# CoderWZW/ARLib

Hardware: AMD Instinct MI355X
Metric: BPR-train interactions/sec (LightGCN d=64 L=3 + BPR + Adam, B=2048) (higher is better)
Workload: dtype f32

## Files before the change

### arlib_amd/csrc/arl_kernels.hip

```cpp
#include <hip/hip_runtime.h>
#include <stdint.h>
#include <math.h>
#include <stdio.h>
#include "arlib_amd.h"
#include "arl_stream.h"
#include "arl_ordered.h"
#include <type_traits>
#include <algorithm>
#include <vector>

namespace {

constexpr int kWave = 64;
constexpr int kBlock = 256;
constexpr int kWavesPerBlock = kBlock / kWave;

__device__ __forceinline__ float wave_sum(float v) {
#pragma unroll
    for (int off = 32; off > 0; off >>= 1) v += __shfl_xor(v, off);
    return v;
}

__device__ __forceinline__ void fma4(float4 &a, float s, const float4 &x) {
    a.x = fmaf(s, x.x, a.x); a.y = fmaf(s, x.y, a.y); a.z = fmaf(s, x.z, a.z); a.w = fmaf(s, x.w, a.w);
// ... 368 lines not shown
    S->cap = (int)cap;
    S->piece_row = w + cap * d;
    S->meta = S->piece_row + cap;
    S->offs = S->meta + 2;
    return true;
}

__global__ __launch_bounds__(kBlock) void tables_sum_kernel(LayerPtrs L, long long n4, float alpha, float4 *__restrict__ out) {
    for (long long t = (long long)blockIdx.x * kBlock + threadIdx.x; t < n4; t += (long long)gridDim.x * kBlock) {
        float4 a = reinterpret_cast<const float4 *>(L.p[0])[t];
        for (int k = 1; k < L.n; ++k) a = add4(a, reinterpret_cast<const float4 *>(L.p[k])[t]);
        out[t] = make_float4(alpha * a.x, alpha * a.y, alpha * a.z, alpha * a.w);
    }
}

__global__ __launch_bounds__(kBlock) void mark_rows_kernel(uint8_t *__restrict__ flags, const int32_t *__restrict__ idx, int n, int value) {
    const int t = blockIdx.x * kBlock + threadIdx.x;
    if (t < n) flags[idx[t]] = (uint8_t)value;
}
__global__ __launch_bounds__(kBlock) void mark_bits_kernel(uint32_t *__restrict__ bits, const int32_t *__restrict__ idx, int n, int set) {
    const int t = blockIdx.x * kBlock + threadIdx.x;
    if (t >= n) return;
    const int i = idx[t];
    if (set) atomicOr(bits + (i >> 5), 1u << (i & 31));
    else atomicAnd(bits + (i >> 5), ~(1u << (i & 31)));
}
__global__ __launch_bounds__(kBlock) void zero_rows_kernel(float *__restrict__ dst, const int32_t *__restrict__ idx, int n, int d) {
    const int lane = threadIdx.x & 63;
    const int t = blockIdx.x * kWavesPerBlock + (threadIdx.x >> 6);
    if (t >= n) return;
    float *o = dst + (size_t)idx[t] * d;
    for (int k = lane; k < d; k += kWave) o[k] = 0.f;
}

template <class RowOf>
__device__ __forceinline__ void stage_rows(int32_t *srows, int c0, int c1, RowOf rowof) {
    for (int j = threadIdx.x; j < c1 - c0; j += kBlock) srows[j] = (int32_t)rowof(c0 + j);
    __syncthreads();
}

__global__ __launch_bounds__(kBlock) void rows_mark_dups_kernel(uint32_t *__restrict__ bits, uint32_t *__restrict__ dup, const int32_t *__restrict__ idx, int n,
                                                                 const float *__restrict__ row_scale) {
    const int t = blockIdx.x * kBlock + threadIdx.x;
    if (t >= n) return;
    if (row_scale && row_scale[t] == 0.f) return;
    const int row = idx[t];
    const uint32_t m = 1u << (row & 31);
    if (atomicOr(bits + (row >> 5), m) & m) atomicOr(dup + (row >> 5), m);
}

template <bool MARK>
__global__ __launch_bounds__(kBlock) void rows_add_ordered_kernel(float *__restrict__ dst, uint8_t *__restrict__ flags, uint32_t *__restrict__ bits,
                                                                   const int32_t *__restrict__ idx, int c0, int c1, int d,
                                                                   const float *__restrict__ src, float scale, const float *__restrict__ row_scale,
                                                                   const uint32_t *__restrict__ dup) {
    extern __shared__ int32_t srows[];
    const int lane = threadIdx.x & 63;
    const int t = c0 + blockIdx.x * kWavesPerBlock + (threadIdx.x >> 6);
    const bool valid = t < c1 && !(row_scale && row_scale[t] == 0.f);
    const int row = valid ? idx[t] : 0;
    float *o = dst + (size_t)row * d;
    const bool fast = valid && dup && !((dup[row >> 5] >> (row & 31)) & 1u);
    if (fast) {
        const float sc = row_scale ? scale * row_scale[t] : scale;
        const float *s = src + (size_t)t * d;
        for (int k = lane; k < d; k += kWave) {
#pragma clang fp contract(off)
            const float c = sc * s[k];
            o[k] = o[k] + c;
        }
        if (MARK && lane == 0) flags[row] = 1;
    }
    if (!__syncthreads_or(valid && !fast)) return;
    stage_rows(srows, c0, c1, [&](int j) { return (row_scale && row_scale[j] == 0.f) ? -1 : idx[j]; });
    if (!valid || fast) return;
    for (int k0 = 0; k0 < d; k0 += 256) {
        float acc[4];
#pragma unroll
        for (int i = 0; i < 4; ++i) { const int k = k0 + 64 * i + lane; acc[i] = k < d ? o[k] : 0.f; }
        const bool owner = ordered_scan_lds_groups(srows, c0, c1, t, row, lane, [&](unsigned long long m, int g0) {
#pragma clang fp contract(off)
            while (m) {
                int tt[4]; float x[4][4], sc[4];
#pragma unroll
                for (int q = 0; q < 4; ++q) {
                    tt[q] = -1;
                    if (m) { tt[q] = g0 + __ffsll((long long)m) - 1; m &= m - 1ull; }
                }
#pragma unroll
                for (int q = 0; q < 4; ++q) {
                    if (tt[q] < 0) continue;
                    const float *s = src + (size_t)tt[q] * d;
                    sc[q] = row_scale ? scale * row_scale[tt[q]] : scale;
#pragma unroll
                    for (int i = 0; i < 4; ++i) { const int k = k0 + 64 * i + lane; x[q][i] = k < d ? s[k] : 0.f; }
                }
#pragma unroll
                for (int q = 0; q < 4; ++q) {
                    if (tt[q] < 0) continue;
#pragma unroll
                    for (int i = 0; i < 4; ++i) { const float c = sc[q] * x[q][i]; acc[i] = acc[i] + c; }
                }
            }
        });
        if (!owner) return;
#pragma unroll
        for (int i = 0; i < 4; ++i) { const int k = k0 + 64 * i + lane; if (k < d) o[k] = acc[i]; }
    }
    if (MARK && lane == 0) {
        flags[row] = 1;
        atomicOr(bits + (row >> 5), 1u << (row & 31));
    }
}
__global__ __launch_bounds__(kBlock) void batch_rows_clear_kernel(float *__restrict__ G, uint8_t *__restrict__ flags, uint32_t *__restrict__ bits,
                                                                   const int32_t *__restrict__ idx, int n, int d, uint32_t *__restrict__ dup) {
    const int lane = threadIdx.x & 63;
    const int t = blockIdx.x * kWavesPerBlock + (threadIdx.x >> 6);
    if (t >= n) return;
    const int row = idx[t];
    float *o = G + (size_t)row * d;
    for (int k = lane; k < d; k += kWave) o[k] = 0.f;
    if (lane == 0) {
        flags[row] = 0;
        atomicAnd(bits + (row >> 5), ~(1u << (row & 31)));
        if (dup) atomicAnd(dup + (row >> 5), ~(1u << (row & 31)));
    }
}

template <int MODE>
int launch_spmm(const arl_csr *A, const float *X, int64_t d, const Epi &ep, hipStream_t st, const uint32_t *xflags = nullptr) {
    if (!A || !X || (A->n_rows > 0 && !A->rowptr) || (A->nnz > 0 && (!A->col || !A->val))) return ARL_E_NULL;
    if (d <= 0 || d > 256 || (d & 3)) return ARL_E_DIM;
    if (A->n_rows < 0 || A->n_rows > 0x7fffffffll || A->nnz > 0x7fffffffll || A->n_chunks > 0x7fffffffll) return ARL_E_RANGE;
    if (A->n_chunks > 0 && (!A->chunk_row || !A->chunk_begin || !A->chunk_end || !A->partial || A->chunk <= 0)) return ARL_E_NULL;
    if (A->n_long > 0 && (!A->long_row || !A->long_first || !A->long_count)) return ARL_E_NULL;
    if ((A->n_chunks > 0) != (A->n_long > 0)) return ARL_E_ARG;
    if (A->n_rows == 0 && A->n_chunks == 0) return ARL_OK;
    CsrDev D;
    D.n_rows = (int)A->n_rows; D.rowptr = A->rowptr; D.col = A->col; D.val = A->val;
    D.chunk = A->chunk; D.n_chunks = (int)A->n_chunks; D.chunk_row = A->chunk_row; D.chunk_begin = A->chunk_begin;
    D.chunk_end = A->chunk_end; D.n_long = (int)A->n_long; D.long_row = A->long_row; D.long_first = A->long_first;
    D.long_count = A->long_count; D.partial = A->partial;
    D.row_tasks = xflags ? reinterpret_cast<const int4 *>(A->row_tasks) : nullptr;
    const long long tasks = (long long)D.n_rows + D.n_chunks;
    const unsigned grid = (unsigned)((tasks + kWavesPerBlock - 1) / kWavesPerBlock);
    const unsigned grid_long = (unsigned)((D.n_long + kWavesPerBlock - 1) / kWavesPerBlock);
    const int di = (int)d;
#define ARL_SPMM_CASE(LPRV)                                                                              \
    do {                                                                                                 \
        if (xflags) hipLaunchKernelGGL((spmm_rows_masked_gpr_kernel<LPRV, MODE>), dim3((unsigned)((tasks + kWavesPerBlock * (kWave / LPRV) - 1) / (kWavesPerBlock * (kWave / LPRV)))), dim3(kBlock), 0, st, D, X, di, ep, xflags); \
        else hipLaunchKernelGGL((spmm_rows_kernel<LPRV, MODE>), dim3(grid), dim3(kBlock), 0, st, D, X, di, ep); \
        ARL_LAUNCH_CHECK();                                                                              \
        if (D.n_long > 0) {                                                                              \
            hipLaunchKernelGGL((spmm_long_rows_kernel<LPRV, MODE>), dim3(grid_long), dim3(kBlock), 0, st, D, di, ep); \
            ARL_LAUNCH_CHECK();                                                                          \
        }                                                                                                \
    } while (0)
    if (d <= 16) ARL_SPMM_CASE(4);
    else if (d <= 32) ARL_SPMM_CASE(8);
    else if (d <= 64) ARL_SPMM_CASE(16);
    else if (d <= 128) ARL_SPMM_CASE(32);
    else ARL_SPMM_CASE(64);
#undef ARL_SPMM_CASE
    return ARL_OK;
}

typedef float f32x32v __attribute__((ext_vector_type(32)));

struct BlockedDev {
    int n_waves;
    const int32_t *wave_ptr;
    const int32_t *wave_rows;
    const int32_t *rec_col;
    const float *rec_val;
    float *partial;
    const uint32_t *xbits;
};

template <int MODE> constexpr int kEpiLoads = MODE == EPI_ADAM ? 4 : 1;
template <int MODE> constexpr int kEpiStores = MODE == EPI_ADAM ? 3 : MODE == EPI_LAYERSUM ? 2 : 1;

template <int MODE>
__device__ __forceinline__ float *spmm_epilogue_table(const Epi &ep, int s) {
    if (MODE == EPI_AXPBY) return ep.Y;
    if (MODE == EPI_LAYERSUM) return s == 0 ? ep.Y : ep.S;
    return s == 0 ? ep.P : s == 1 ? ep.M : ep.V;
}

template <int MODE, int CPL>
__device__ __forceinline__ void spmm_epilogue_math(const Epi &ep, bool zr, float rs, const float *a, const float (&in)[kEpiLoads<MODE>][CPL],
                                                   float (&out)[kEpiStores<MODE>][CPL]) {
#pragma unroll
    for (int c = 0; c < CPL; ++c) {
#pragma clang fp contract(off)
        if constexpr (MODE == EPI_AXPBY) {
            float y = (ep.rscale ? ep.alpha * rs : ep.alpha) * a[c];
            if (zr) y = fmaf(ep.beta, in[0][c], y);
            out[0][c] = y;
        } else if constexpr (MODE == EPI_LAYERSUM) {
            out[0][c] = a[c];
            out[1][c] = in[0][c] + a[c];
        } else {
            float g = ep.alpha * a[c];
            if (zr) g = fmaf(ep.beta, in[0][c], g);
            float p = in[1][c], m = in[2][c], v = in[3][c];
            m = m + (g - m) * ep.w1;
            v = fmaf(ep.w2 * g, g, v * ep.b2);
            const float denom = sqrtf(v) / ep.bc2_sqrt + ep.eps;
            p = fmaf(-ep.step_size, m / denom, p);
            out[0][c] = p; out[1][c] = m; out[2][c] = v;
        }
    }
}

template <int MODE, int CPL, int LD>
__device__ __forceinline__ void spmm_epilogue1(const Epi &ep, int row, bool zr, float rs, int lane, const float *a) {
    const size_t o = (size_t)row * LD;
    const unsigned lo = lane * CPL;
    float in[kEpiLoads<MODE>][CPL], out[kEpiStores<MODE>][CPL];
#pragma unroll
    for (int c = 0; c < CPL; ++c) {
        in[0][c] = 0.f;
        if constexpr (MODE == EPI_LAYERSUM) in[0][c] = (ep.S_in + o)[lo + c];
        else if (zr) in[0][c] = (ep.Z + o)[lo + c];
        if constexpr (MODE == EPI_ADAM) { in[1][c] = (ep.P + o)[lo + c]; in[2][c] = (ep.M + o)[lo + c]; in[3][c] = (ep.V + o)[lo + c]; }
    }
    spmm_epilogue_math<MODE, CPL>(ep, zr, rs, a, in, out);
#pragma unroll
    for (int s = 0; s < kEpiStores<MODE>; ++s) {
        if (MODE == EPI_LAYERSUM && s == 0 && !ep.Y) continue;
        float *dst = spmm_epilogue_table<MODE>(ep, s) + o;
#pragma unroll
        for (int c = 0; c < CPL; ++c) {
            if (MODE == EPI_AXPBY) __builtin_nontemporal_store(out[s][c], dst + (lo + c));
            else dst[lo + c] = out[s][c];
        }
    }
}

template <int MODE, int K, int CPL, int LD>
__device__ __forceinline__ void spmm_group_load(const Epi &ep, int my_row, unsigned zmask, int safe_row, int r0, int lane, float (&in)[K][kEpiLoads<MODE>][CPL]) {
    const unsigned lo = lane * CPL;
    const size_t so = (size_t)safe_row * LD;
    if constexpr (MODE != EPI_LAYERSUM) {
#pragma unroll
        for (int i = 0; i < K; ++i)
#pragma unroll
            for (int c = 0; c < CPL; ++c) in[i][0][c] = 0.f;
        if (ep.Z) {
#pragma unroll
            for (int i = 0; i < K; ++i) {
                const int row = __builtin_amdgcn_readlane(my_row, r0 + i);
                const float *z = ((zmask >> (r0 + i)) & 1u) ? ep.Z + (size_t)row * LD : ep.Z + so;
#pragma unroll
                for (int c = 0; c < CPL; ++c) in[i][0][c] = z[lo + c];
            }
        }
    }
    if constexpr (MODE != EPI_AXPBY) {
#pragma unroll
        for (int i = 0; i < K; ++i) {
            const int row = __builtin_amdgcn_readlane(my_row, r0 + i);
            const size_t o = (size_t)row * LD;
#pragma unroll
            for (int c = 0; c < CPL; ++c) {
                if constexpr (MODE == EPI_LAYERSUM) in[i][0][c] = (row >= 0 ? ep.S_in + o : ep.S_in + so)[lo + c];
                else {
                    in[i][1][c] = (row >= 0 ? ep.P + o : ep.P + so)[lo + c];
                    in[i][2][c] = (row >= 0 ? ep.M + o : ep.M + so)[lo + c];
                    in[i][3][c] = (row >= 0 ? ep.V + o : ep.V + so)[lo + c];
                }
            }
        }
    }
}

template <int MODE, int K, int CPL, int LD>
__device__ __forceinline__ void spmm_group_store(const Epi &ep, float *partial, int my_row, int r0, int lane, const float (&a)[K][CPL],
                                                 const float (&out)[K][kEpiStores<MODE>][CPL]) {
    const unsigned lo = lane * CPL;
#pragma unroll
    for (int s = 0; s < kEpiStores<MODE>; ++s) {
        if (MODE == EPI_LAYERSUM && s == 0 && !ep.Y) continue;
        float *tab = spmm_epilogue_table<MODE>(ep, s);
#pragma unroll
        for (int i = 0; i < K; ++i) {
            const int row = __builtin_amdgcn_readlane(my_row, r0 + i);
            const bool plain = row >= 0;
            float *dst = plain ? tab + (size_t)row * LD : partial + (size_t)(plain ? 0 : -row - 2) * (64 * CPL);
#pragma unroll
            for (int c = 0; c < CPL; ++c) {
                const float y = plain ? out[i][s][c] : a[i][c];
                if (MODE == EPI_AXPBY) __builtin_nontemporal_store(y, dst + (lo + c));
                else dst[lo + c] = y;
            }
        }
    }
}

template <int UNR, bool MASKED> constexpr bool kEpiGrouped = MASKED || UNR == 16;
template <int MODE, bool MASKED> constexpr int kEpiGroup = MODE == EPI_ADAM ? 2 : MASKED ? 8 : 4;

constexpr int kMaskedUnr = 8;

constexpr int kMaxMergedSets = 4;
struct BlockedSetsDev {
    int n;
    int block_end[kMaxMergedSets];
    BlockedDev s[kMaxMergedSets];
};

template <int RPW, int MODE, int UNR, int CPL, int LD = 64 * CPL, bool MASKED = false, typename PLAN = BlockedDev>
__global__ __launch_bounds__(kBlock) void spmm_blocked64_kernel(PLAN plan, const float *__restrict__ X, Epi ep) {
    static_assert(RPW == 16 || RPW == 32, "accumulators are 32-register vectors");
    static_assert(CPL == 1 || CPL == 2, "d = 64 (one column per lane) or d = 128 (two adjacent columns per lane)");
    const int lane = threadIdx.x & 63;
    BlockedDev P;
    int w;
    if constexpr (std::is_same<PLAN, BlockedSetsDev>::value) {
        P = plan.s[0];
        int b0 = 0;
#pragma unroll
        for (int i = 1; i < kMaxMergedSets; ++i)
            if (i < plan.n && (int)blockIdx.x >= plan.block_end[i - 1]) { P = plan.s[i]; b0 = plan.block_end[i - 1]; }
        w = ((int)blockIdx.x - b0) * (blockDim.x >> 6) + (threadIdx.x >> 6);
    } else {
        P = plan;
        w = blockIdx.x * (blockDim.x >> 6) + (threadIdx.x >> 6);
    }
    if (w >= P.n_waves) return;
    f32x32v acc[CPL];
#pragma unroll
    for (int c = 0; c < CPL; ++c)
#pragma unroll
        for (int r = 0; r < 32; ++r) acc[c][r] = 0.f;
    const int begin = P.wave_ptr[w], end = P.wave_ptr[w + 1];
    constexpr bool GROUPED = kEpiGrouped<UNR, MASKED>;
    int my_row = -1;
    if (GROUPED && lane < RPW) my_row = P.wave_rows[(size_t)w * RPW + lane];
    const float *xl = X + lane * CPL;
    if (MASKED) {
        int c0 = 0, c1 = 0; unsigned w0 = 0;
        if (begin < end) c0 = __builtin_nontemporal_load(P.rec_col + begin + lane);
        if (begin + 64 < end) c1 = __builtin_nontemporal_load(P.rec_col + begin + 64 + lane);
        if (begin < end) w0 = P.xbits[((unsigned)c0 & 0xffffffu) >> 5];
        for (int base = begin; base < end; base += 64) {
            const int c_cur = c0; const unsigned w_cur = w0;
            c0 = c1;
            if (base + 128 < end) c1 = __builtin_nontemporal_load(P.rec_col + base + 128 + lane);
            if (base + 64 < end) w0 = P.xbits[((unsigned)c0 & 0xffffffu) >> 5];
            unsigned long long hits = __ballot((w_cur >> (c_cur & 31)) & 1u);
            while (hits) {
                float x[kMaskedUnr][CPL], vs[kMaskedUnr]; int cs[kMaskedUnr], js[kMaskedUnr];
#pragma unroll
                for (int t = 0; t < kMaskedUnr; ++t) {
                    js[t] = hits ? __builtin_ctzll(hits) : -1;
                    hits &= hits - 1ull;
                    if (js[t] < 0) continue;
                    cs[t] = __builtin_amdgcn_readlane(c_cur, js[t]);
                    vs[t] = P.rec_val[base + js[t]];
                    const float *src = xl + (size_t)(cs[t] & 0xffffff) * LD;
                    if (CPL == 2) { const float2 v2 = *reinterpret_cast<const float2 *>(src); x[t][0] = v2.x; x[t][CPL - 1] = v2.y; }
                    else x[t][0] = src[0];
                }
#pragma unroll
                for (int t = 0; t < kMaskedUnr; ++t) {
                    if (js[t] < 0) continue;
                    const int slot = ((unsigned)cs[t] >> 24) & 31;
#pragma unroll
                    for (int c = 0; c < CPL; ++c) acc[c][slot] = fmaf(vs[t], x[t][c], acc[c][slot]);
                }
            }
        }
    } else {
    int rc = 0; float rv = 0.f;
    if (begin < end) { rc = __builtin_nontemporal_load(P.rec_col + begin + lane); rv = __builtin_nontemporal_load(P.rec_val + begin + lane); }
    for (int base = begin; base < end; base += 64) {
        const int c_cur = rc; const float v_cur = rv;
        if (base + 64 < end) { rc = __builtin_nontemporal_load(P.rec_col + base + 64 + lane); rv = __builtin_nontemporal_load(P.rec_val + base + 64 + lane); }
#pragma unroll
        for (int j = 0; j < 64; j += UNR) {
            float x[UNR][CPL]; int cs[UNR];
#pragma unroll
            for (int t = 0; t < UNR; ++t) {
                cs[t] = __builtin_amdgcn_readlane(c_cur, j + t);
                const float *src = xl + (size_t)(cs[t] & 0xffffff) * LD;
                if (CPL == 2) { const float2 v2 = *reinterpret_cast<const float2 *>(src); x[t][0] = v2.x; x[t][CPL - 1] = v2.y; }
                else x[t][0] = src[0];
            }
#pragma unroll
            for (int t = 0; t < UNR; ++t) {
                const int slot = ((unsigned)cs[t] >> 24) & 31;
                const float v = __uint_as_float((unsigned)__builtin_amdgcn_readlane((int)__float_as_uint(v_cur), j + t));
#pragma unroll
                for (int c = 0; c < CPL; ++c) acc[c][slot] = fmaf(v, x[t][c], acc[c][slot]);
            }
        }
    }
    }
    auto row_epilogue = [&](int row, bool zr, float rs, const float *a) {
        if (row >= 0) spmm_epilogue1<MODE, CPL, LD>(ep, row, zr, rs, lane, a);
        else if (row < -1) {
            float *dst = P.partial + ((size_t)(-row - 2) * 64 + lane) * CPL;
#pragma unroll
            for (int c = 0; c < CPL; ++c) dst[c] = a[c];
        }
    };
    if constexpr (!GROUPED) {
#pragma unroll
        for (int r = 0; r < RPW; ++r) {
            const int row = P.wave_rows[w * RPW + r];
            float a[CPL];
#pragma unroll
            for (int c = 0; c < CPL; ++c) a[c] = acc[c][r];
            const bool zr = row >= 0 && MODE != EPI_LAYERSUM && ep.Z && (!ep.zflags || ep.zflags[row]);
            const float rs = (row >= 0 && MODE == EPI_AXPBY && ep.rscale) ? ep.rscale[row] : 0.f;
            row_epilogue(row, zr, rs, a);
        }
    } else {
    bool my_zr = false; float my_rs = 0.f;
    if (my_row >= 0) {
        if (MODE == EPI_AXPBY && ep.rscale) my_rs = ep.rscale[my_row];
        if (MODE != EPI_LAYERSUM) my_zr = ep.Z && (!ep.zflags || ep.zflags[my_row]);
    }
    const unsigned zmask = (unsigned)__ballot(my_zr);
    const unsigned long long rows = __ballot(my_row >= 0), pads = __ballot(my_row == -1);
    constexpr int K = kEpiGroup<MODE, MASKED>, NG = RPW / K;
    static_assert(RPW % K == 0, "whole groups");
    const int n_grouped = rows ? __builtin_ctzll(pads) / K : 0;
    if (n_grouped > 0) {
        const int safe_row = __builtin_amdgcn_readlane(my_row, __builtin_ctzll(rows));
        float in[2][K][kEpiLoads<MODE>][CPL];
        spmm_group_load<MODE, K, CPL, LD>(ep, my_row, zmask, safe_row, 0, lane, in[0]);
#pragma unroll
        for (int g = 0; g < NG; ++g) {
            if (g + 1 < NG) spmm_group_load<MODE, K, CPL, LD>(ep, my_row, zmask, safe_row, (g + 1) * K, lane, in[(g + 1) & 1]);
            float a[K][CPL], out[K][kEpiStores<MODE>][CPL];
#pragma unroll
            for (int i = 0; i < K; ++i) {
                const int r = g * K + i;
#pragma unroll
                for (int c = 0; c < CPL; ++c) a[i][c] = acc[c][r];
                const float rs = __uint_as_float((unsigned)__builtin_amdgcn_readlane((int)__float_as_uint(my_rs), r));
                spmm_epilogue_math<MODE, CPL>(ep, (zmask >> r) & 1u, rs, a[i], in[g & 1][i], out[i]);
            }
            spmm_group_store<MODE, K, CPL, LD>(ep, P.partial, my_row, g * K, lane, a, out);
            if (g + 1 == n_grouped) break;
        }
    }
#pragma nounroll
    for (int r = n_grouped * K; r < RPW; ++r) {
        float a[CPL];
#pragma unroll
        for (int c = 0; c < CPL; ++c) a[c] = acc[c][r];
        row_epilogue(__builtin_amdgcn_readlane(my_row, r), (zmask >> r) & 1u, __uint_as_float((unsigned)__builtin_amdgcn_readlane((int)__float_as_uint(my_rs), r)), a);
    }
    }
}

template <int RPW, int MODE, int UNR, int CPL, int LD>
static int launch_blocked64(dim3 grid, dim3 block, hipStream_t st, const BlockedDev &D, const float *X, const Epi &ep) {
    if (D.xbits) {
        if constexpr (MODE == EPI_AXPBY) hipLaunchKernelGGL((spmm_blocked64_kernel<RPW, MODE, UNR, CPL, LD, true>), grid, block, 0, st, D, X, ep);
        else return ARL_E_ARG;
    } else hipLaunchKernelGGL((spmm_blocked64_kernel<RPW, MODE, UNR, CPL, LD, false>), grid, block, 0, st, D, X, ep);
    ARL_LAUNCH_CHECK();
    return ARL_OK;
}

static int blocked_set_check(const arl_blocked *P) {
    if (P->n_waves < 0 || P->n_waves > 0x7fffffffll / 64) return ARL_E_RANGE;
    if (P->rows_per_wave != 16 && P->rows_per_wave != 32) return ARL_E_ARG;
    if (P->n_waves == 0) return ARL_OK;
    if (!P->wave_ptr || !P->wave_rows || !P->rec_col || !P->rec_val) return ARL_E_NULL;
    if (P->n_split < 0 || P->n_split > 0x7fffffffll) return ARL_E_RANGE;
    if (P->n_split > 0 && (!P->split_row || !P->split_first || !P->split_count || !P->partial)) return ARL_E_NULL;
    const int64_t wpg = P->waves_per_group ? P->waves_per_group : kWavesPerBlock;
    if (wpg != 1 && wpg != 2 && wpg != 4) return ARL_E_ARG;
    if (P->loads_in_flight != 16 && P->loads_in_flight != 32) return ARL_E_ARG;
    return ARL_OK;
}

static BlockedDev blocked_dev(const arl_blocked *P, const uint32_t *xbits) {
    return {(int)P->n_waves, P->wave_ptr, P->wave_rows, P->rec_col, P->rec_val, P->partial, xbits};
}

template <int MODE, int LD>
static int launch_blocked_set(const arl_blocked *P, const float *X, const Epi &ep, hipStream_t st, const uint32_t *xbits) {
    const BlockedDev D = blocked_dev(P, xbits);
    const int64_t wpg = P->waves_per_group ? P->waves_per_group : kWavesPerBlock;
    const dim3 grid((unsigned)((P->n_waves + wpg - 1) / wpg)), block((unsigned)(wpg * kWave));
    if (P->rows_per_wave == 16) return launch_blocked64<16, MODE, 16, 1, LD>(grid, block, st, D, X, ep);
    if (P->loads_in_flight == 16) return launch_blocked64<32, MODE, 16, 1, LD>(grid, block, st, D, X, ep);
    return launch_blocked64<32, MODE, 32, 1, LD>(grid, block, st, D, X, ep);
}

template <int MODE>
static int launch_split_combine(int64_t n_split, const int32_t *row, const int32_t *first, const int32_t *count, float *partial, const Epi &ep, hipStream_t st) {
    if (n_split <= 0) return ARL_OK;
    CsrDev C = {};
    C.n_long = (int)n_split; C.long_row = row; C.long_first = first; C.long_count = count; C.partial = partial;
    const unsigned grid_long = (unsigned)((C.n_long + kWavesPerBlock - 1) / kWavesPerBlock);
    hipLaunchKernelGGL((spmm_long_rows_kernel<16, MODE>), dim3(grid_long), dim3(kBlock), 0, st, C, 64, ep);
    ARL_LAUNCH_CHECK();
    return ARL_OK;
}

static Epi epi_half(const Epi &ep, int half) {
    Epi e2 = ep;
    e2.ld = 128;
    const int off = 64 * half;
    if (e2.Z) e2.Z += off;
    if (e2.Y) e2.Y += off;
    if (e2.S_in) e2.S_in += off;
    if (e2.S) e2.S += off;
    if (e2.P) e2.P += off;
    if (e2.M) e2.M += off;
    if (e2.V) e2.V += off;
    return e2;
}

template <int MODE>
int launch_spmm_blocked(const arl_blocked *P, const float *X, int64_t d, const Epi &ep, hipStream_t st, const uint32_t *xbits = nullptr) {
    if (!P || !X) return ARL_E_NULL;
    if (d != 64 && d != 128) return ARL_E_DIM;
    if (int rc = blocked_set_check(P)) return rc;
    if (P->n_waves == 0) return ARL_OK;
    for (int half = 0; half < (d == 128 ? 2 : 1); ++half) {
        const Epi e2 = d == 128 ? epi_half(ep, half) : ep;
        int rc = d == 128 ? launch_blocked_set<MODE, 128>(P, X + 64 * half, e2, st, xbits) : launch_blocked_set<MODE, 64>(P, X, e2, st, xbits);
        if (rc != ARL_OK) return rc;
        rc = launch_split_combine<MODE>(P->n_split, P->split_row, P->split_first, P->split_count, P->partial, e2, st);
        if (rc != ARL_OK) return rc;
    }
    return ARL_OK;
}

template <int LD>
static int launch_masked_sets(const arl_blocked *sets, const int *order, int m, const float *X, const Epi &ep, hipStream_t st, const uint32_t *xbits) {
    BlockedSetsDev S = {};
    S.n = m;
    int64_t blocks = 0, wpg = kWavesPerBlock;
    for (int i = 0; i < m; ++i) wpg = std::min<int64_t>(wpg, sets[order[i]].waves_per_group ? sets[order[i]].waves_per_group : kWavesPerBlock);
    for (int i = 0; i < m; ++i) {
        const arl_blocked *P = sets + order[i];
        blocks += (P->n_waves + wpg - 1) / wpg;
        if (blocks > 0x7fffffffll) return ARL_E_RANGE;
        S.block_end[i] = (int)blocks; S.s[i] = blocked_dev(P, xbits);
    }
    for (int i = m; i < kMaxMergedSets; ++i) { S.block_end[i] = (int)blocks; S.s[i] = S.s[0]; }
    const dim3 grid((unsigned)blocks), block((unsigned)(wpg * kWave));
    if (sets[order[0]].rows_per_wave == 16) hipLaunchKernelGGL((spmm_blocked64_kernel<16, EPI_AXPBY, 16, 1, LD, true, BlockedSetsDev>), grid, block, 0, st, S, X, ep);
    else hipLaunchKernelGGL((spmm_blocked64_kernel<32, EPI_AXPBY, 16, 1, LD, true, BlockedSetsDev>), grid, block, 0, st, S, X, ep);
    ARL_LAUNCH_CHECK();
    return ARL_OK;
}

template <int MODE>
int launch_spmm_blocked_sets(const arl_blocked *sets, int64_t n_sets, int64_t first, const arl_blocked_hop *hop, const float *X, int64_t d, const Epi &ep,
                             hipStream_t st, const uint32_t *xbits = nullptr) {
    if (!X || (n_sets > 0 && !sets)) return ARL_E_NULL;
    if (d != 64 && d != 128) return ARL_E_DIM;
    if (n_sets < 0 || n_sets > 0x7fffffffll || first < 0 || first > n_sets) return ARL_E_RANGE;
    if (xbits && MODE != EPI_AXPBY) return ARL_E_ARG;
    int64_t skipped = 0, n_split = 0;
    std::vector<int> run;
    bool one_rpw = true;
    for (int64_t k = 0; k < n_sets; ++k) {
        if (int rc = blocked_set_check(sets + k)) return rc;
        if (sets[k].n_split < 0 || sets[k].n_split > 0x7fffffffll) return ARL_E_RANGE;
        if (k < first) { skipped += sets[k].n_split; continue; }
        n_split += sets[k].n_split;
        if (sets[k].n_waves == 0) { if (sets[k].n_split) return ARL_E_ARG; continue; }
        if (!run.empty() && sets[k].rows_per_wave != sets[run[0]].rows_per_wave) one_rpw = false;
        run.push_back((int)k);
    }
    if (run.empty()) return ARL_OK;
    if (n_split > 0) {
        if (!hop || !hop->split_row || !hop->split_first || !hop->split_count || !hop->partial) return ARL_E_NULL;
        if (skipped + n_split > hop->n_split) return ARL_E_ARG;
    }
    const int m = (int)run.size();
    const bool merged = xbits && m > 1 && m <= kMaxMergedSets && one_rpw;
    if (merged && hop && hop->stream_len)
        std::stable_sort(run.begin(), run.end(), [&](int a, int b) { return hop->stream_len[a] > hop->stream_len[b]; });
    for (int half = 0; half < (d == 128 ? 2 : 1); ++half) {
        const Epi e2 = d == 128 ? epi_half(ep, half) : ep;
        const float *Xh = X + 64 * half;
        int rc = ARL_OK;
        if (merged) {
            if constexpr (MODE == EPI_AXPBY) rc = d == 128 ? launch_masked_sets<128>(sets, run.data(), m, Xh, e2, st, xbits) : launch_masked_sets<64>(sets, run.data(), m, Xh, e2, st, xbits);
        } else {
            for (int i = 0; i < m && rc == ARL_OK; ++i)
                rc = d == 128 ? launch_blocked_set<MODE, 128>(sets + run[i], Xh, e2, st, xbits) : launch_blocked_set<MODE, 64>(sets + run[i], Xh, e2, st, xbits);
        }
        if (rc != ARL_OK) return rc;
        if (n_split > 0) {
            rc = launch_split_combine<MODE>(n_split, hop->split_row + skipped, hop->split_first + skipped, hop->split_count + skipped, hop->partial, e2, st);
            if (rc != ARL_OK) return rc;
        }
    }
    return ARL_OK;
}

__global__ __launch_bounds__(kBlock) void row_dinv_kernel(int n_rows, const int32_t *__restrict__ rowptr,
                                                           const float *__restrict__ w, float *__restrict__ dinv) {
    const int lane = threadIdx.x & 63;
    const int r = blockIdx.x * kWavesPerBlock + (threadIdx.x >> 6);
    if (r >= n_rows) return;
    float s = 0.f;
    for (int e = rowptr[r] + lane; e < rowptr[r + 1]; e += kWave) s += w[e];
    s = wave_sum(s);
    if (lane == 0) dinv[r] = s > 0.f ? 1.0f / sqrtf(s) : 0.f;
}

__global__ __launch_bounds__(kBlock) void norm_vals_kernel(int n_rows, const int32_t *__restrict__ rowptr,
                                                            const int32_t *__restrict__ col, const float *__restrict__ w,
                                                            const float *__restrict__ dinv, float *__restrict__ val) {
    const int lane = threadIdx.x & 63;
    const int r = blockIdx.x * kWavesPerBlock + (threadIdx.x >> 6);
    if (r >= n_rows) return;
    const float dr = dinv[r];
    for (int e = rowptr[r] + lane; e < rowptr[r + 1]; e += kWave) val[e] = (dr * w[e]) * dinv[col[e]];
}

__global__ __launch_bounds__(kBlock) void norm_vals_coo_kernel(long long nnz, const int32_t *__restrict__ erow, const int32_t *__restrict__ col,
                                                                const float *__restrict__ w, const float *__restrict__ dinv, float *__restrict__ val) {
    const long long e0 = ((long long)blockIdx.x * kBlock + threadIdx.x) * 4;
    if (e0 + 3 < nnz) {
        const int4 r = *reinterpret_cast<const int4 *>(erow + e0), c = *reinterpret_cast<const int4 *>(col + e0);
        const float4 ww = *reinterpret_cast<const float4 *>(w + e0);
        float4 o;
        o.x = (dinv[r.x] * ww.x) * dinv[c.x]; o.y = (dinv[r.y] * ww.y) * dinv[c.y];
        o.z = (dinv[r.z] * ww.z) * dinv[c.z]; o.w = (dinv[r.w] * ww.w) * dinv[c.w];
        *reinterpret_cast<float4 *>(val + e0) = o;
    } else {
        for (long long e = e0; e < nnz; ++e) val[e] = (dinv[erow[e]] * w[e]) * dinv[col[e]];
    }
}

__global__ __launch_bounds__(kBlock) void bpr_fwd_kernel(const float *__restrict__ emb, int d, long long item_off,
                                                          const int32_t *__restrict__ ui, const int32_t *__restrict__ pi,
                                                          const int32_t *__restrict__ ni, int B, float b_norm, float *__restrict__ ws) {
    const int lane = threadIdx.x & 63;
    const int b = blockIdx.x * kWavesPerBlock + (threadIdx.x >> 6);
    if (b >= B) return;
    const float *u = emb + (size_t)ui[b] * d, *p = emb + (size_t)(item_off + pi[b]) * d, *n = emb + (size_t)(item_off + ni[b]) * d;
    float ps = 0.f, ns = 0.f, uu = 0.f, pp = 0.f;
    for (int k = lane; k < d; k += kWave) {
        const float uk = u[k], pk = p[k], nk = n[k];
        ps = fmaf(uk, pk, ps); ns = fmaf(uk, nk, ns); uu = fmaf(uk, uk, uu); pp = fmaf(pk, pk, pp);
    }
    ps = wave_sum(ps); ns = wave_sum(ns); uu = wave_sum(uu); pp = wave_sum(pp);
    if (lane == 0) {
        const float x = ps - ns;
        const float s = 1.0f / (1.0f + expf(-x));
        ws[b] = -(s * (1.0f - s)) / ((1e-7f + s) * b_norm);
        ws[B + b] = -logf(1e-7f + s);
        ws[2 * B + b] = uu;
        ws[3 * B + b] = pp;
    }
}

__global__ __launch_bounds__(kBlock) void bpr_finalize_kernel(int B, float reg, const float *__restrict__ ws, float *__restrict__ out, int raw_sums) {
    __shared__ float sh[3][kBlock];
    float a = 0.f, b = 0.f, c = 0.f;
    for (int i = threadIdx.x; i < B; i += kBlock) { a += ws[B + i]; b += ws[2 * B + i]; c += ws[3 * B + i]; }
    sh[0][threadIdx.x] = a; sh[1][threadIdx.x] = b; sh[2][threadIdx.x] = c;
    __syncthreads();
    for (int s = kBlock / 2; s > 0; s >>= 1) {
        if ((int)threadIdx.x < s) {
            sh[0][threadIdx.x] += sh[0][threadIdx.x + s]; sh[1][threadIdx.x] += sh[1][threadIdx.x + s]; sh[2][threadIdx.x] += sh[2][threadIdx.x + s];
        }
        __syncthreads();
    }
// ... 4058 lines not shown
```

Before: 335,500.

## Batch masked SpMM over four-chunk windows with branchless gather issue

Reworks the masked SpMM path so each iteration processes a window of four 64-record chunks. Column and bitmask words are prefetched a full window ahead, and hits from all four chunks are pooled into fixed-size unrolled gather batches. Out-of-range slots are padded with a safe column and a zero weight, so there are no per-slot branches. The intent is to fill gather batches and hide load latency when hit density per chunk is low, at the cost of more registers and some wasted padded loads.

```diff
diff --git a/arlib_amd/csrc/arl_kernels.hip b/arlib_amd/csrc/arl_kernels.hip
--- a/arlib_amd/csrc/arl_kernels.hip
+++ b/arlib_amd/csrc/arl_kernels.hip
@@ -694,6 +694,7 @@
 template <int MODE, bool MASKED> constexpr int kEpiGroup = MODE == EPI_ADAM ? 2 : MASKED ? 8 : 4;
 
 constexpr int kMaskedUnr = 8;
+constexpr int kMaskedWin = 4;
 
 constexpr int kMaxMergedSets = 4;
 struct BlockedSetsDev {
@@ -732,37 +733,64 @@
     if (GROUPED && lane < RPW) my_row = P.wave_rows[(size_t)w * RPW + lane];
     const float *xl = X + lane * CPL;
     if (MASKED) {
-        int c0 = 0, c1 = 0; unsigned w0 = 0;
-        if (begin < end) c0 = __builtin_nontemporal_load(P.rec_col + begin + lane);
-        if (begin + 64 < end) c1 = __builtin_nontemporal_load(P.rec_col + begin + 64 + lane);
-        if (begin < end) w0 = P.xbits[((unsigned)c0 & 0xffffffu) >> 5];
-        for (int base = begin; base < end; base += 64) {
-            const int c_cur = c0; const unsigned w_cur = w0;
-            c0 = c1;
-            if (base + 128 < end) c1 = __builtin_nontemporal_load(P.rec_col + base + 128 + lane);
-            if (base + 64 < end) w0 = P.xbits[((unsigned)c0 & 0xffffffu) >> 5];
-            unsigned long long hits = __ballot((w_cur >> (c_cur & 31)) & 1u);
-            while (hits) {
-                float x[kMaskedUnr][CPL], vs[kMaskedUnr]; int cs[kMaskedUnr], js[kMaskedUnr];
-#pragma unroll
-                for (int t = 0; t < kMaskedUnr; ++t) {
-                    js[t] = hits ? __builtin_ctzll(hits) : -1;
-                    hits &= hits - 1ull;
-                    if (js[t] < 0) continue;
-                    cs[t] = __builtin_amdgcn_readlane(c_cur, js[t]);
-                    vs[t] = P.rec_val[base + js[t]];
+        const int sb = __builtin_amdgcn_readfirstlane(begin), se = __builtin_amdgcn_readfirstlane(end);
+        if (sb < se) {
+        constexpr int W = kMaskedWin, U = kMaskedUnr;
+        const int32_t *rc = P.rec_col + lane;
+        const int last = se - 64;
+        int c0[W], c1[W]; unsigned w0[W];
+#pragma unroll
+        for (int k = 0; k < W; ++k) c0[k] = __builtin_nontemporal_load(rc + (sb + k * 64 < se ? sb + k * 64 : last));
+#pragma unroll
+        for (int k = 0; k < W; ++k) c1[k] = __builtin_nontemporal_load(rc + (sb + (W + k) * 64 < se ? sb + (W + k) * 64 : last));
+#pragma unroll
+        for (int k = 0; k < W; ++k) w0[k] = P.xbits[((unsigned)c0[k] & 0xffffffu) >> 5];
+        for (int base = sb; base < se; base += 64 * W) {
+            int c_cur[W]; unsigned w_cur[W];
+#pragma unroll
+            for (int k = 0; k < W; ++k) { c_cur[k] = c0[k]; w_cur[k] = w0[k]; c0[k] = c1[k]; }
+#pragma unroll
+            for (int k = 0; k < W; ++k) c1[k] = __builtin_nontemporal_load(rc + (base + (2 * W + k) * 64 < se ? base + (2 * W + k) * 64 : last));
+#pragma unroll
+            for (int k = 0; k < W; ++k) w0[k] = P.xbits[((unsigned)c0[k] & 0xffffffu) >> 5];
+            unsigned long long hits[W]; int n = 0;
+#pragma unroll
+            for (int k = 0; k < W; ++k) {
+                hits[k] = __ballot((w_cur[k] >> (c_cur[k] & 31)) & 1u);
+                if (base + k * 64 >= se) hits[k] = 0;
+                n += __builtin_popcountll(hits[k]);
+            }
+            if (n == 0) continue;
+            const int c_safe = __builtin_amdgcn_readfirstlane(c_cur[0]);
+            int kb = 0, c_sel = c_cur[0]; unsigned long long h = hits[0];
+            float x[U][CPL], vs[U]; int cs[U];
+            auto issue = [&]() {
+#pragma unroll
+                for (int t = 0; t < U; ++t) {
+#pragma unroll
+                    for (int k = 1; k < W; ++k)
+                        if (!h && kb < k) { kb = k; h = hits[k]; c_sel = c_cur[k]; }
+                    const bool ok = h != 0;
+                    const int j = ok ? __builtin_ctzll(h) : 0;
+                    h &= h - 1ull;
+                    cs[t] = ok ? __builtin_amdgcn_readlane(c_sel, j) : c_safe;
+                    vs[t] = P.rec_val[ok ? base + kb * 64 + j : base];
                     const float *src = xl + (size_t)(cs[t] & 0xffffff) * LD;
                     if (CPL == 2) { const float2 v2 = *reinterpret_cast<const float2 *>(src); x[t][0] = v2.x; x[t][CPL - 1] = v2.y; }
                     else x[t][0] = src[0];
                 }
-#pragma unroll
-                for (int t = 0; t < kMaskedUnr; ++t) {
-                    if (js[t] < 0) continue;
+            };
+            auto consume = [&](int m) {
+#pragma unroll
+                for (int t = 0; t < U; ++t) {
                     const int slot = ((unsigned)cs[t] >> 24) & 31;
-#pragma unroll
-                    for (int c = 0; c < CPL; ++c) acc[c][slot] = fmaf(vs[t], x[t][c], acc[c][slot]);
+                    const float v = t < m ? vs[t] : 0.f;
+#pragma unroll
+                    for (int c = 0; c < CPL; ++c) acc[c][slot] = fmaf(v, t < m ? x[t][c] : 0.f, acc[c][slot]);
                 }
-            }
+            };
+            for (; n > 0; n -= U) { issue(); consume(n); }
+        }
         }
     } else {
     int rc = 0; float rv = 0.f;
```

Result: slower. 332,200 (-1.0%).
